# PraveenVora/pinot

Measured on AMD Instinct MI355X. Metric: rows/sec scanned + %HBM roofline, filter+GROUP BY SUM at 1/2/4/8 GPUs, higher is better.
Workload: dtype int64; 1 GPU; adanalytics_readme_query; rows_per_gpu=1000000000, segments_per_gpu=100, parallelism=segment-sharded dp1, RCCL reduce of partial aggregates, groups=8, matched_docs_rank0=118

## Files before the change

### include/pinot_amd.h

```cpp
#ifndef PINOT_AMD_H_
#define PINOT_AMD_H_

#include <stdint.h>

#ifdef __cplusplus
extern "C" {
#endif

#define PA_ABI_VERSION 5

#define PA_MAX_LEAVES 16
#define PA_MAX_OPS 48
#define PA_MAX_GROUP_BY 8
#define PA_MAX_AGGS 16
#define PA_MAX_ORDER_BY 8
#define PA_MAX_SELECT_COLUMNS 64
#define PA_MAX_SELECT_ROWS 65536
#define PA_MAX_AGG_FILTERS 8
#define PA_MAX_EXPRS 8
#define PA_MAX_EXPR_OPS 16
#define PA_MAX_EXPR_REGS 8
#define PA_MAX_EXPR_COLUMNS 8

#define PA_OK 0
// ... 344 lines not shown
                        void* stream);

int pa_query_key_layout(const pa_query* q, int32_t* hashed, int32_t* shifts);
int32_t pa_query_key_words(const pa_query* q);

int pa_query_stats(const pa_query* q, uint64_t* staged_bytes, uint64_t* num_docs,
                   uint64_t* num_tiles);

int32_t pa_query_column_staged(const pa_query* q, int32_t column_id);
int32_t pa_query_num_eager_literals(const pa_query* q);
int32_t pa_query_lane_major(const pa_query* q);
int32_t pa_query_dense_packed(const pa_query* q);
int32_t pa_query_count_free_emit(const pa_query* q);
int32_t pa_query_eq_prefilter(const pa_query* q);
int32_t pa_query_stream_nt(const pa_query* q);
int32_t pa_query_partition_keys(const pa_query* q);
int pa_query_plan(const pa_query* q, int32_t* strategy, int32_t* steps, int32_t* dma_slots, int32_t* ring,
                  int32_t* wg_per_cu, int32_t* grid, int32_t* lds_bytes);

void pa_query_destroy(pa_query* q);

#ifdef __cplusplus
}
#endif

#endif
```

### pinot_amd/_lib.py

```python
import ctypes
import os

HERE = os.path.dirname(os.path.abspath(__file__))
LIB_PATH = os.path.join(HERE, "libpinot_amd.so")

PA_MAX_LEAVES = 16
PA_MAX_OPS = 48
PA_MAX_GROUP_BY = 8
PA_MAX_AGGS = 16
PA_MAX_ORDER_BY = 8
PA_MAX_SELECT_COLUMNS = 64
PA_MAX_SELECT_ROWS = 65536
PA_MAX_AGG_FILTERS = 8
PA_MAX_EXPRS, PA_MAX_EXPR_OPS, PA_MAX_EXPR_REGS, PA_MAX_EXPR_COLUMNS = 8, 16, 8, 8
PA_EXPR_DOUBLE, PA_EXPR_LONG = 0, 1
PA_EXPR_ARG_REG, PA_EXPR_ARG_COL, PA_EXPR_ARG_F64, PA_EXPR_ARG_I64 = range(4)
PA_EXPR_LOAD_COL, PA_EXPR_ADD, PA_EXPR_SUB, PA_EXPR_MUL, PA_EXPR_DIV, PA_EXPR_MOD, PA_EXPR_ABS, PA_EXPR_CEIL, \
    PA_EXPR_FLOOR, PA_EXPR_D2L, PA_EXPR_L2D, PA_EXPR_TCONV_DIV, PA_EXPR_TCONV_MUL = range(13)

PA_OK, PA_EINVAL, PA_EHIP, PA_ENOMEM, PA_EUNSUPPORTED = 0, -1, -2, -3, -4
PA_INT, PA_LONG, PA_FLOAT, PA_DOUBLE, PA_STRING, PA_BYTES = range(6)
PA_LEAF_DICT_RANGE, PA_LEAF_DICT_SET, PA_LEAF_RAW_RANGE, PA_LEAF_MV_DICT_RANGE, PA_LEAF_MV_DICT_SET, PA_LEAF_RAW_SET = range(6)
PA_OP_LEAF, PA_OP_AND, PA_OP_OR, PA_OP_NOT = range(4)
PA_AGG_COUNT, PA_AGG_SUM, PA_AGG_MIN, PA_AGG_MAX, PA_AGG_DISTINCTCOUNTHLL, PA_AGG_COUNT_MV, PA_AGG_DISTINCTCOUNT, \
# ... 38 lines not shown
ABI_VERSION = 5

EXPORTED = [
    "pa_abi_version", "pa_device_count", "pa_set_device", "pa_last_error", "pa_host_alloc", "pa_host_free",
    "pa_segment_create", "pa_segment_add_sv_dict_column", "pa_segment_add_mv_dict_column",
    "pa_segment_add_raw_column", "pa_segment_num_docs", "pa_segment_device_bytes", "pa_segment_destroy",
    "pa_query_create", "pa_query_set_tuning", "pa_query_results_invalid", "pa_query_bind_segment",
    "pa_query_bind_value_remap", "pa_query_prepare", "pa_query_num_keys",
    "pa_query_set_selection", "pa_query_bind_order_remap", "pa_query_fetch_selection",
    "pa_query_selection_segment_docs", "pa_query_selection_counters",
    "pa_query_set_distinct", "pa_query_fetch_distinct",
    "pa_query_set_agg_filters", "pa_query_fetch_lane_counts", "pa_query_lane_docs",
    "pa_query_set_expressions",
    "pa_query_execute", "pa_query_reset", "pa_query_scan", "pa_query_num_eager_literals", "pa_query_lane_major",
    "pa_query_dense_packed", "pa_query_count_free_emit", "pa_query_eq_prefilter", "pa_query_stream_nt",
    "pa_query_partition_keys",
    "pa_query_accumulator_bytes", "pa_query_set_accumulator_buffer", "pa_query_num_sections", "pa_query_section",
    "pa_query_fetch", "pa_query_fetch_trimmed", "pa_query_fetch_histogram", "pa_query_percentiles",
    "pa_query_fetch_time_rows", "pa_query_time_row_form", "pa_query_matched_docs", "pa_query_key_layout", "pa_query_limit_trimming",
    "pa_query_num_groups_limit_reached", "pa_query_stats", "pa_query_leaf_bitmap_words", "pa_query_leaf_bitmaps",
    "pa_bitmap_counts_scratch_bytes", "pa_bitmap_counts", "pa_query_filter_counts",
    "pa_query_plan", "pa_query_column_staged", "pa_query_leap_leaf", "pa_query_leap_counts",
    "pa_query_execution_stats",
    "pa_query_row_bytes", "pa_query_pack_rows", "pa_query_merge_rows", "pa_query_key_words", "pa_query_destroy",
]


class PinotAmdError(RuntimeError):
    pass


# ... 132 lines not shown
        "pa_query_set_agg_filters": (ctypes.c_int, [vp, ctypes.POINTER(AggFilterSpec)]),
        "pa_query_fetch_lane_counts": (ctypes.c_int, [vp, vp, i64, vp]),
        "pa_query_lane_docs": (ctypes.c_int, [vp, vp]),
        "pa_query_set_expressions": (ctypes.c_int, [vp, ctypes.POINTER(ExprSpec)]),
        "pa_query_prepare": (ctypes.c_int, [vp]),
        "pa_query_num_keys": (i64, [vp]),
        "pa_query_execute": (ctypes.c_int, [vp, vp]),
        "pa_query_reset": (ctypes.c_int, [vp, vp]),
        "pa_query_scan": (ctypes.c_int, [vp, vp]),
        "pa_query_num_eager_literals": (i32, [vp]),
        "pa_query_lane_major": (i32, [vp]),
        "pa_query_dense_packed": (i32, [vp]),
        "pa_query_count_free_emit": (i32, [vp]),
        "pa_query_eq_prefilter": (i32, [vp]),
        "pa_query_stream_nt": (i32, [vp]),
        "pa_query_partition_keys": (i32, [vp]),
        "pa_query_accumulator_bytes": (u64, [vp]),
        "pa_query_set_accumulator_buffer": (ctypes.c_int, [vp, vp, u64]),
        "pa_query_num_sections": (i32, [vp]),
        "pa_query_section": (vp, [vp, i32, ctypes.POINTER(i32), ctypes.POINTER(i64)]),
        "pa_query_fetch": (i64, [vp, vp, i64, vp, vp, vp]),
        "pa_query_fetch_trimmed": (i64, [vp, vp, ctypes.POINTER(TrimSpec), i64, vp, vp, vp, ctypes.POINTER(i64)]),
        "pa_query_fetch_histogram": (i64, [vp, vp, i32, i64, i64, vp, vp, vp]),
        "pa_query_percentiles": (ctypes.c_int, [vp, vp, i32, i64, i32, vp, vp]),
        "pa_query_fetch_time_rows": (ctypes.c_int, [vp, vp, i32, i64, i32, vp, vp, vp, vp]),
        "pa_query_time_row_form": (i32, [vp, i32]),
        "pa_query_matched_docs": (i64, [vp]),
        "pa_query_key_layout": (ctypes.c_int, [vp, ctypes.POINTER(i32), ctypes.POINTER(i32)]),
        "pa_query_limit_trimming": (i32, [vp]),
        "pa_query_num_groups_limit_reached": (ctypes.c_int64, [vp]),
# ... 48 lines not shown
```

### pinot_amd/build.py

```python
import os
import re
import subprocess
import sys
import time
from concurrent.futures import ThreadPoolExecutor

HERE = os.path.dirname(os.path.abspath(__file__))
CSRC = os.path.join(HERE, "csrc")
LIB = os.path.join(HERE, "libpinot_amd.so")
SOURCES = ["pa_scan_lane_lm.hip", "pa_scan_std.hip", "pa_scan_part_mv.hip", "pa_scan_part_b.hip", "pa_scan_lane_raw.hip",
           "pa_scan_gdense.hip", "pa_scan_global.hip", "pa_scan_lane_dict.hip", "pa_kernels.hip", "pa_scan_part_a.hip",
           "pa_scan_filtered.hip", "pa_scan_expr.hip", "pa_scan_trow.hip", "pa_stats.hip", "pa_stats_host.hip", "pa_scan_lane_sm.hip", "pa_scan_distinct.hip",
           "pa_scan_select.hip", "pa_plan.hip",
           "pa_jit.hip", "pa_plan_kernels.hip", "pa_select.hip", "pa_distinct.hip", "pa_fetch.hip", "pa_capi.hip",
           "pa_compact.hip", "pa_segment.hip", "pa_hist.hip", "pa_prep.hip", "pa_launch_scan.hip", "pa_merge.hip",
           "pa_pve.hip", "pa_trim.hip"]
HEADERS = sorted(f for f in os.listdir(CSRC) if f.endswith(".h")) + [os.path.join("..", "..", "include", "pinot_amd.h")]
FLAGS = ["--offload-arch=gfx950", "-O3", "-fPIC", "-shared", "-munsafe-fp-atomics", "-std=c++17",
         "-Wall", "-Wno-unused-function"]
JIT_SOURCES = ["gdl_jit.hip", "pve_jit.hip"]
JIT_ABI = "pa_jit_abi.h"
_INCLUDE = re.compile(r'^\s*#\s*include\s+"([^"]+)"', re.M)


def _deps(path, seen=None):
    seen = set() if seen is None else seen
    if path in seen or not os.path.exists(path):
        return seen
    seen.add(path)
    for inc in _INCLUDE.findall(open(path, errors="replace").read()):
        for d in (os.path.dirname(path), CSRC, os.path.join(HERE, "..", "include")):
            cand = os.path.normpath(os.path.join(d, inc))
            if os.path.exists(cand):
                _deps(cand, seen)
                break
# ... 83 lines not shown
```

### pinot_amd/csrc/pa_capi.hip

```cpp
#include "pa_host.h"

extern "C" {

pa_query* pa_query_create(const pa_query_spec* spec, int32_t num_segments) {
  if (!spec || num_segments < 0) {
    fail(PA_EINVAL, "bad query spec");
    return nullptr;
  }
  if (spec->num_leaves < 0 || spec->num_leaves > PA_MAX_LEAVES || spec->num_ops < 0 || spec->num_ops > PA_MAX_OPS ||
      spec->num_group_by < 0 || spec->num_group_by > PA_MAX_GROUP_BY || spec->num_aggs < 0 ||
      spec->num_aggs > PA_MAX_AGGS) {
    fail(PA_EINVAL, "query spec counts out of range");
    return nullptr;
  }
  pa_query* q = new pa_query();
  q->spec = *spec;
  q->nseg = num_segments;
  q->segs.assign(num_segments, nullptr);
  q->leaf_params.resize(num_segments);
  q->luts.resize(num_segments);
  q->remaps.resize(num_segments);
  q->has_remap.resize(num_segments);
  q->vremaps.assign(num_segments, std::vector<std::vector<int32_t>>(spec->num_aggs));
  return q;
// ... 269 lines not shown
    rc = plan_limit_buffers(q, P, cus, total_tiles);
    if (rc) return rc;
  }
  rc = alloc_leaps(q, P);
  if (rc) return rc;
  rc = upload_descriptors(q);
  if (rc) return rc;
  if (q->trow_wide) {
    rc = dev_alloc(q->dq_pass2, sizeof(DevQuery));
    if (rc) return rc;
    DevQuery h2 = q->hq;
    h2.trow_pass = 2;
    PA_HIP(hipMemcpy(q->dq_pass2.p, &h2, sizeof(DevQuery), hipMemcpyHostToDevice));
  }
  if (!q->is_distinct) rc = jit_plan(q, P, cus);
  if (rc) return rc;
  if (q->is_distinct) {
    rc = distinct_plan(q);
    if (rc) return rc;
  }
  rc = pve_plan(q, P, cus);
  if (rc) return rc;
  PA_HIP(hipDeviceSynchronize());
  q->prepared = true;
  return PA_OK;
}

int64_t pa_query_num_keys(const pa_query* q) { return q ? q->num_keys : -1; }

int pa_query_reset(pa_query* q, void* stream) {
// ... 120 lines not shown
      PA_HIP(launch_scan(q->emit_h_strat, q->steps, 0, q->grid, q->emit_h_lds, (const DevQuery*)q->dq_h.p,
                         (const DevSeg*)q->dsegs.p, plans, ps, st));
    PA_HIP(launch_part_agg(q->part_vk, (const DevQuery*)q->dq.p, ps, q->hq.num_parts, q->hq.pv, q->hq.v_fmt <= V_FMT_ID,
                           q->tune.passc_v16, q->part_lds_c, st));
    PA_HIP(hipEventRecord(a->last, st));
    a->last_stream = st;
    a->used = true;
    return PA_OK;
  }
  if (q->jit_fn) {
    void* pa = q->jit_args.p;
    void* ps = q->jit_segs.p;
    void* params[] = {&pa, &ps};
    PA_HIP(hipModuleLaunchKernel(q->jit_fn, q->jit_grid, 1, 1, q->jit_waves * kWave, 1, 1, q->jit_lds, st, params,
                                 nullptr));
    return PA_OK;
  }
  PartScratch none{};
  PA_HIP(launch_scan(q->strategy, q->steps, q->lane_major, q->grid, q->lds_bytes, (const DevQuery*)q->dq.p,
                     (const DevSeg*)q->dsegs.p, (const LmSegPlan*)q->dplans.p, none, st));
  if (q->trow_wide)
    PA_HIP(launch_scan(q->strategy, q->steps, q->lane_major, q->grid, q->lds_bytes, (const DevQuery*)q->dq_pass2.p,
                       (const DevSeg*)q->dsegs.p, (const LmSegPlan*)q->dplans.p, none, st));
  q->leap_searched = false;
  return PA_OK;
}

int pa_query_execute(pa_query* q, void* stream) {
  const int rc = pa_query_reset(q, stream);
  return rc ? rc : pa_query_scan(q, stream);
// ... 80 lines not shown
  return q->sections[section].ptr;
}

int pa_query_stats(const pa_query* q, uint64_t* staged_bytes, uint64_t* num_docs, uint64_t* num_tiles) {
  if (!q) return fail(PA_EINVAL, "null query");
  if (staged_bytes) *staged_bytes = q->staged_bytes;
  if (num_docs) *num_docs = q->num_docs;
  if (num_tiles) *num_tiles = q->num_tiles;
  return PA_OK;
}

int pa_query_plan(const pa_query* q, int32_t* strategy, int32_t* steps, int32_t* dma_slots, int32_t* ring,
                  int32_t* wg_per_cu, int32_t* grid, int32_t* lds_bytes) {
  if (!q || !q->prepared) return fail(PA_EINVAL, "query not prepared");
  if (strategy)
    *strategy = q->jit_fn ? (q->jit_waves >= 16 ? STRAT_GDENSE_LM16 : STRAT_GDENSE_LM8)
                          : (q->partitioned ? STRAT_PEMIT : q->strategy);
  if (steps) *steps = q->steps;
  if (dma_slots) *dma_slots = q->dma_slots;
  if (ring) *ring = q->plan_ring;
  if (wg_per_cu) *wg_per_cu = q->plan_wg;
  if (grid) *grid = q->grid;
  if (lds_bytes) *lds_bytes = q->lds_bytes;
  return PA_OK;
}

int32_t pa_query_num_eager_literals(const pa_query* q) { return q && q->prepared ? q->num_eager : -1; }

int32_t pa_query_time_row_form(const pa_query* q, int32_t agg) {
  if (!q || !q->prepared || agg < 0 || agg >= q->spec.num_aggs) return -1;
  return q->trow_form[agg];
}

int32_t pa_query_lane_major(const pa_query* q) { return q && q->prepared ? q->lane_major : -1; }
int32_t pa_query_eq_prefilter(const pa_query* q) { return q && q->prepared ? q->eq_prefilter : -1; }
int32_t pa_query_stream_nt(const pa_query* q) { return q && q->prepared ? q->stream_nt : -1; }
int32_t pa_query_count_free_emit(const pa_query* q) { return q && q->prepared ? (q->pve.fn ? (q->pvh.fn ? 2 : 1) : 0) : -1; }
int32_t pa_query_partition_keys(const pa_query* q) {
  if (!q || !q->prepared) return -1;
  if (!q->partitioned || q->hq.pv == 0) return 0;
  return q->hq.part_kr_v ? q->hq.part_kr_v : (int32_t)1 << q->hq.kshift_v;
}
int32_t pa_query_dense_packed(const pa_query* q) {
  return q && q->prepared ? (q->jit_fn ? 2 : (q->dense_packed ? 1 : 0)) : -1;
}

int32_t pa_query_column_staged(const pa_query* q, int32_t column_id) {
  if (!q || !q->prepared || q->nseg == 0) return -1;
  for (size_t sl = 0; sl < q->slot_cols.size(); ++sl)
    if (q->slot_cols[sl] == column_id) {
      if (q->jit_fn) return std::count(q->jit_cols.begin(), q->jit_cols.end(), (int)sl) ? 1 : 0;
      return q->hsegs[0].cols[sl].lds_off >= 0 ? 1 : 0;
    }
  return -1;
}

int64_t pa_query_matched_docs(const pa_query* q) { return q && q->prepared ? q->last_matched : -1; }

int32_t pa_query_limit_trimming(const pa_query* q) {
// ... 19 lines not shown
```

### pinot_amd/csrc/pa_host.h

```cpp
#pragma once
#include <hip/hip_runtime.h>
#include <hip/hiprtc.h>

#include <algorithm>
#include <array>
#include <cstdio>
#include <cstdlib>
#include <cmath>
#include <cstring>
#include <functional>
#include <map>
#include <mutex>
#include <numeric>
#include <string>
#include <utility>
#include <vector>

#include "pa_device.h"
#include "pa_launch.h"
#include "pa_jit_abi.h"
#include "pa_tuning.h"

using namespace pa;

// ... 189 lines not shown

  DevQuery hq;
  std::vector<DevSeg> hsegs;
  DevBuf dq, dsegs, dplans;
  void* host_acc = nullptr;
  DevBuf fetch_blocks, fetch_stage;
  void* fetch_host = nullptr;
  DevBuf trim_buf;
  int lane_major = 0;
  int eq_prefilter = 0;
  int stream_nt = 0;
  int dense_packed = 0;
  hipFunction_t jit_fn = nullptr;
  int jit_waves = 0, jit_grid = 0, jit_lds = 0, jit_nd = 16, jit_nseg = 0, jit_classes = 0, jit_slots = 0;
  std::vector<int> jit_cols;
  DevBuf jit_args, jit_segs;
  struct PveStream {
    hipFunction_t fn = nullptr;
    int waves = 0, grid = 0, lds = 0, cr = 0, parts = 0, bin_shift = 5;
    int64_t chunks = 0;
    DevBuf args, segs, buf;
    size_t o_table = 0, o_hist = 0, o_used = 0, o_off = 0, o_base = 0, o_index = 0, o_tot = 0;
  } pve, pvh;
  int has_mv = 0;
  bool hashed = false;
  int key_words = 1;
  int64_t ht_slots = 0;
  int key_shift[PA_MAX_GROUP_BY] = {0};
  int keys_section = -1;
  bool partitioned = false;
// ... 200 lines not shown
int plan_scratch(pa_query* q, const Prep& P);
int plan_walk(pa_query* q, const Prep& P);
int plan_limit_buffers(pa_query* q, const Prep& P, int cus, int64_t total_tiles);
int upload_descriptors(pa_query* q);
PartScratch scratch_of(const pa_query* q, void* base);
size_t leap_header_bytes(const pa_query* q);
int plan_leaps(pa_query* q, const Prep& P);
int alloc_leaps(pa_query* q, const Prep& P);
int select_validate(pa_query* q);
int select_plan(pa_query* q);
int select_reset(pa_query* q, hipStream_t st);
int distinct_key_space(pa_query* q, Prep& P);
int distinct_plan(pa_query* q);
int jit_plan(pa_query* q, const Prep& P, int cus);
void jit_fill_pointers(pa_query* q, JitArgs& a);
void pve_fill_pointers(const pa_query::PveStream& st, unsigned long long* matched, PveArgs& a);
int pve_plan(pa_query* q, const Prep& P, int cus);
```

### pinot_amd/csrc/pa_jit.hip

```cpp
#include "pa_host.h"

static const char* kGdlJitSrc =
#include "gdl_jit_src.inc"
    ;

namespace {
std::mutex g_jit_mu;
struct JitEntry {
  hipModule_t mod = nullptr;
  hipFunction_t fn = nullptr;
};
std::map<std::string, JitEntry> g_jit_cache;

std::string int_list(const std::vector<int>& v) {
  std::string r = "{";
  for (size_t i = 0; i < v.size(); ++i) r += (i ? "," : "") + std::to_string(v[i]);
  return r + "}";
}

hipFunction_t jit_compile(const std::vector<std::string>& defs, const char* src = kGdlJitSrc,
                          const char* name = "gdl_jit") {
  int dev = 0;
  (void)hipGetDevice(&dev);
  std::string key = std::to_string(dev) + " " + name;
// ... 54 lines not shown

struct JitSum {
  int col = 0;
  int w = 0;
  bool table = false;
  bool shared = true;
  bool offs = false;
  int64_t base = 0, step = 1;
  std::vector<int64_t> aoff;
  int max_card = 0;
};
}

int jit_plan(pa_query* q, const Prep& P, int cus) {
  q->jit_fn = nullptr;
  q->jit_cols.clear();
  const pa_query_spec& s = q->spec;
  if (q->nseg == 0 || s.num_group_by != 1 || !P.gd_box_ok || P.gd_box || q->hq.leap_mode || q->partitioned ||
      q->limit_mode || q->limit_walk || q->hashed)
    return PA_OK;
  const Tuning& tn = q->tune;
  if ((s.flags & PA_QF_NO_JIT) || tn.debug_emit) return PA_OK;
  if (s.flags & (PA_QF_NO_DENSE_GROUP | PA_QF_FORCE_GLOBAL | PA_QF_FORCE_LDS | PA_QF_LAZY_POST | PA_QF_NO_LANE_MAJOR |
                 PA_QF_STEPS16 | PA_QF_DEBUG_STREAM_ONLY | PA_QF_NO_GDENSE_LM | PA_QF_NO_GD_PACK))
    return PA_OK;
  const int nl_all = (int)q->literals.size();
  if (q->num_eager != nl_all) return PA_OK;
  for (int li = 0; li < nl_all; ++li) {
    const int kind = s.leaves[q->literals[li].leaf].kind;
    if (kind != PA_LEAF_DICT_RANGE && kind != PA_LEAF_DICT_SET) return PA_OK;
// ... 435 lines not shown
  PA_HIP(hipMemcpy(q->jit_args.p, &a, sizeof(a), hipMemcpyHostToDevice));
  PA_HIP(hipMemcpy(q->jit_segs.p, js.data(), sizeof(JitSeg) * js.size(), hipMemcpyHostToDevice));
  q->jit_fn = fn;
  q->jit_waves = W;
  q->jit_nd = ND;
  q->jit_lds = (int)lds;
  q->jit_grid = G;
  q->jit_nseg = ni;
  q->jit_classes = (int)classes.size();
  q->jit_slots = nslot;
  q->jit_cols = cols;
  PLAN_LOG("gdl_jit: W %d ND %d RS %d RR %d ring %d lmax %d segdrain %d classes %zu slots %d (%zu B) segments %d/%d "
           "ktab %d kib %d lds %zu drain %d",
           W, ND, RS, RR, ring_n, lmax, (int)segdrain, classes.size(), nslot, slot_b, ni, q->nseg, (int)ktab, (int)kib,
           lds, drain);
  return PA_OK;
}

static const char* kPveJitSrc =
#include "pve_jit_src.inc"
    ;


void pve_fill_pointers(const pa_query::PveStream& st, unsigned long long* matched, PveArgs& a) {
  char* b = (char*)st.buf.p;
  a.recs = (uint32_t*)b;
  a.table = (uint32_t*)(b + st.o_table);
  a.hist = (uint32_t*)(b + st.o_hist);
  a.used = (uint32_t*)(b + st.o_used);
  a.matched = matched;
// ... 317 lines not shown
```

### pinot_amd/csrc/pa_jit_abi.h

```cpp
#pragma once

constexpr int kJitMax = 6;
constexpr int kJitMaxGb = 4;

struct JitSeg {
  unsigned long long src[kJitMax];
  long long first_tile;
  int num_docs, num_tiles;
  unsigned int lo_t[kJitMax], hi_t[kJitMax];
  int cls;
  int lbase, lspan;
  int gofs;
  int aoff[kJitMax];
  unsigned long long ktab;
  unsigned long long lut[kJitMax];
  unsigned long long tab[kJitMax];
  int lut_words[kJitMax];
  int tab_n[kJitMax];
  int ktab_n;
  unsigned int neg;
};
struct JitArgs {
  long long total_tiles;
  int nseg, nkeys, key_lo, key_span, xcd_major, pad;
  long long key_stride;
  unsigned long long* matched;
  unsigned long long* count;
  long long* sum[kJitMax];
  int sum_long[kJitMax];
  long long base[kJitMax], step[kJitMax];
};
static_assert(sizeof(JitSeg) == 48 + 8 + 8 + 48 + 16 + 24 + 8 + 48 + 48 + 24 + 24 + 8, "JitSeg layout");
static_assert(sizeof(JitArgs) == 8 + 24 + 8 + 8 + 8 + 48 + 24 + 48 + 48, "JitArgs layout");

struct PveSeg {
  unsigned long long src[kJitMax];
  long long first_tile;
  int num_docs, num_tiles;
  unsigned int lo_t[kJitMax], hi_t[kJitMax];
  unsigned long long admit;
  unsigned long long raw;
  unsigned long long mv_off;
  unsigned long long mv_words;
  unsigned long long hlut;
  int koff[kJitMaxGb];
  unsigned long long ktab[kJitMaxGb];
  int voff, vtab_n;
  unsigned long long vtab;
};
// ... 13 lines not shown
```

### pinot_amd/csrc/pa_tuning.h

```cpp
#pragma once
#include <cstdint>
#include <cstring>

#define PA_TUNINGS(X)                                                                                                  \
                                                                                  \
  X(gdl_w, -1, 8, 16, 0)                                                                                               \
  X(gdl_nd, -1, 8, 16, 0)                                                                                              \
  X(gdl_rs, -1, 1, 2, 0)                                                                                               \
                                                                                        \
  X(gdl_rr, -1, 1, 64, 0)                                                                                              \
                    \
  X(gdl_ring, -1, 2, 4, 0)                                                                                             \
         \
  X(gdl_dbg, 0, 0, 3, 1)                                                                                               \
                                      \
  X(pve_nd, -1, 8, 16, 0)                                                                                              \
         \
  X(pve_bs, -1, 16, 32, 0)                                                                                             \
                                                                              \
  X(pve_q, -1, 0, 1, 0)                                                                                                \
   \
  X(pve_ring, -1, 2, 4, 0)                                                                                             \
              \
  X(pve_hrun, -1, 0, 1, 0)                                                                                             \
                       \
  X(pve_hb, -1, 1, 8, 0)                                                                                               \
                                    \
  X(pve_dbg, 0, 0, 2, 1)                                                                                               \
                                                               \
  X(passc_v16, -1, 0, 1, 0)                                                                                            \
                                                                      \
  X(walk_tab, 1, 0, 1, 0)                                                                                              \
               \
  X(debug_emit, 0, 0, 127, 1)                                                                                          \
                                \
  X(eq_prefilter, -1, 0, 1, 0)                                                                                         \
                                                                                            \
  X(stream_nt, -1, 0, 1, 0)                                                                                            \
        \
  X(scan_grid, -1, 1, 4096, 0)                                                                                         \
                                                                    \
  X(reset_fused, -1, 0, 1, 0)                                                                                          \
         \
  X(select_scratch_mib, 256, 1, 16384, 0)                                                                              \
                                                    \
  X(select_cap, -1, 2, 131072, 0)                                                                                      \
     \
  X(distinct_lds, 1, 0, 2, 0)                                                                                          \
                                                                                 \
  X(filtered_lds, -1, 0, 1, 0)                                                                                         \
                                                    \
  X(expr_lds, -1, 0, 1, 0)                                                                                             \
    \
// ... 36 lines not shown
```

### pinot_amd/engine.py

```python
import ctypes
import dataclasses
import threading
from dataclasses import dataclass, field
from typing import Dict, List, Optional

import numpy as np

from . import _lib as L
from . import predicate as P
from . import query as Q
from . import transform as T
from .hll import HyperLogLog, hash_value
from .java_hash import java_hash_code
from .optimizer import optimize_filter
from .segment import Segment

_VTYPE = {"INT": L.PA_INT, "LONG": L.PA_LONG, "FLOAT": L.PA_FLOAT, "DOUBLE": L.PA_DOUBLE, "STRING": L.PA_STRING}


class UnsupportedQuery(L.PinotAmdError):
    pass


def column_ids_for(segment: Segment) -> Dict[str, int]:
# ... 699 lines not shown
        names = ("strategy", "steps", "dma_slots", "ring", "wg_per_cu", "grid", "lds_bytes")
        out["plan"] = {n: v.value for n, v in zip(names, vals)}
        code = out["plan"]["strategy"]
        out["plan"]["strategy"] = {0: "lds", 1: "global", 2: "partitioned", 4: "lane", 5: "lane", 6: "lane", 7: "lane",
                                    8: "lds_dense", 9: "lds_dense", 10: "lds_dense", 11: "lds_dense", 12: "lds_dense",
                                    14: "lds_dense", 15: "lds_dense", 128: "select", 129: "distinct",
                                    130: "distinct", 131: "filtered", 132: "filtered", 133: "expr", 134: "expr",
                                    135: "time_rows", 136: "time_rows"}[code]
        out["plan"]["variant"] = STRATEGY_VARIANTS.get(code, str(code))
        out["plan"]["eager_literals"] = int(L.lib().pa_query_num_eager_literals(self.handle))
        out["plan"]["lane_major"] = int(L.lib().pa_query_lane_major(self.handle))
        out["plan"]["dense_packed"] = int(L.lib().pa_query_dense_packed(self.handle))
        out["plan"]["count_free_emit"] = int(L.lib().pa_query_count_free_emit(self.handle))
        out["plan"]["eq_prefilter"] = int(L.lib().pa_query_eq_prefilter(self.handle))
        out["plan"]["stream_nt"] = int(L.lib().pa_query_stream_nt(self.handle))
        out["plan"]["partition_keys"] = int(L.lib().pa_query_partition_keys(self.handle))
        out["plan"]["limit_trimming"] = int(L.lib().pa_query_limit_trimming(self.handle))
        out["plan"]["results_invalid"] = int(L.lib().pa_query_results_invalid(self.handle))
        out["plan"]["time_row_form"] = {i: int(L.lib().pa_query_time_row_form(self.handle, i))
                                        for i, (t, _, _) in enumerate(self.pa_aggs) if t in TIME_ROW_AGGS}
        return out

    def fetch_arrays(self, stream=None, pooled=False, trim_spec=None):
        lib = L.lib()
        alloc = (lambda slot, n, dt: OUTPUT_POOL.array(slot, n, dt)) if pooled else (lambda slot, n, dt: np.empty(n, dt))
        cap = 1 if not self.query.group_by else min(self.num_keys, 1 << 16)
        if trim_spec is not None:
            cap = max(1, min(self.num_keys, int(trim_spec.trim)))
            total = ctypes.c_int64(0)
        elif self.query.group_by and self.num_keys > 1 << 16:
# ... 679 lines not shown
```

Before: 2580 billion rows/s.

## Add JIT-compiled equality-scan kernel with SWAR prefilter and lazy survivor aggregation

Adds a new JIT-compiled kernel, eqs_jit, for queries whose first leaf is an equality on a packed dictionary column and whose aggregates are int/long SUMs. Packed bit tiles stream into LDS through a ring of global_load_lds DMA buffers. A branch-free SWAR borrow trick tests whether any value in a word can match and skips tiles with no candidates. Only surviving docs decode the lazy leaves, group-by keys and sum columns straight from global memory and update them with atomics. The aim is to cut ALU and decode work on a very selective filter so the scan runs near HBM bandwidth, at the cost of extra planning, JIT compile time and a separate code path.

```diff
diff --git a/include/pinot_amd.h b/include/pinot_amd.h
--- a/include/pinot_amd.h
+++ b/include/pinot_amd.h
@@ -382,6 +382,7 @@
 int32_t pa_query_count_free_emit(const pa_query* q);
 int32_t pa_query_eq_prefilter(const pa_query* q);
 int32_t pa_query_stream_nt(const pa_query* q);
+int32_t pa_query_eq_jit(const pa_query* q);
 int32_t pa_query_partition_keys(const pa_query* q);
 int pa_query_plan(const pa_query* q, int32_t* strategy, int32_t* steps, int32_t* dma_slots, int32_t* ring,
                   int32_t* wg_per_cu, int32_t* grid, int32_t* lds_bytes);
diff --git a/pinot_amd/_lib.py b/pinot_amd/_lib.py
--- a/pinot_amd/_lib.py
+++ b/pinot_amd/_lib.py
@@ -76,7 +76,7 @@
     "pa_query_set_expressions",
     "pa_query_execute", "pa_query_reset", "pa_query_scan", "pa_query_num_eager_literals", "pa_query_lane_major",
     "pa_query_dense_packed", "pa_query_count_free_emit", "pa_query_eq_prefilter", "pa_query_stream_nt",
-    "pa_query_partition_keys",
+    "pa_query_eq_jit", "pa_query_partition_keys",
     "pa_query_accumulator_bytes", "pa_query_set_accumulator_buffer", "pa_query_num_sections", "pa_query_section",
     "pa_query_fetch", "pa_query_fetch_trimmed", "pa_query_fetch_histogram", "pa_query_percentiles",
     "pa_query_fetch_time_rows", "pa_query_time_row_form", "pa_query_matched_docs", "pa_query_key_layout", "pa_query_limit_trimming",
@@ -239,6 +239,7 @@
         "pa_query_count_free_emit": (i32, [vp]),
         "pa_query_eq_prefilter": (i32, [vp]),
         "pa_query_stream_nt": (i32, [vp]),
+        "pa_query_eq_jit": (i32, [vp]),
         "pa_query_partition_keys": (i32, [vp]),
         "pa_query_accumulator_bytes": (u64, [vp]),
         "pa_query_set_accumulator_buffer": (ctypes.c_int, [vp, vp, u64]),
diff --git a/pinot_amd/build.py b/pinot_amd/build.py
--- a/pinot_amd/build.py
+++ b/pinot_amd/build.py
@@ -18,7 +18,7 @@
 HEADERS = sorted(f for f in os.listdir(CSRC) if f.endswith(".h")) + [os.path.join("..", "..", "include", "pinot_amd.h")]
 FLAGS = ["--offload-arch=gfx950", "-O3", "-fPIC", "-shared", "-munsafe-fp-atomics", "-std=c++17",
          "-Wall", "-Wno-unused-function"]
-JIT_SOURCES = ["gdl_jit.hip", "pve_jit.hip"]
+JIT_SOURCES = ["gdl_jit.hip", "pve_jit.hip", "eqs_jit.hip"]
 JIT_ABI = "pa_jit_abi.h"
 _INCLUDE = re.compile(r'^\s*#\s*include\s+"([^"]+)"', re.M)
 
diff --git a/pinot_amd/csrc/eqs_jit.hip b/pinot_amd/csrc/eqs_jit.hip
--- /dev/null
+++ b/pinot_amd/csrc/eqs_jit.hip
@@ -0,0 +1,388 @@
+typedef unsigned int u32;
+typedef unsigned long long u64;
+typedef long long i64;
+typedef __attribute__((address_space(3))) u32 l32;
+typedef __attribute__((address_space(3))) u64 l64;
+typedef const __attribute__((address_space(1))) u32 g32;
+typedef const __attribute__((address_space(1))) int gi32;
+typedef const __attribute__((address_space(1))) i64 gi64;
+typedef __attribute__((address_space(1))) u64 gu64;
+
+#include "pa_jit_abi.h"
+
+#ifndef JIT_DBG
+#define JIT_DBG 0
+#endif
+constexpr int W = JIT_W, R = JIT_RING, IMG = JIT_IMG, NCLS = JIT_NCLS, NLZ = JIT_NLZ, NG = JIT_NG, NA = JIT_NA;
+constexpr int kNB[NCLS] = JIT_NB;
+constexpr int TD = 2048;
+constexpr u32 REG = 16;
+static_assert(R >= 2 && R <= 8, "2..8 tile images per wave");
+static_assert(NCLS >= 1 && NCLS <= 4, "1..4 width classes");
+static_assert(NLZ <= kJitMax && NG <= kJitMaxGb && NA <= kJitMax, "shape beyond the JIT descriptors");
+
+typedef const __attribute__((address_space(4))) JitArgs CA;
+typedef const __attribute__((address_space(4))) EqsHdr CH;
+typedef const __attribute__((address_space(4))) EqsSeg CS;
+
+__device__ __forceinline__ u32 lds_addr(const void* p) { return (u32)(unsigned long)(const l32*)p; }
+template <class T>
+__device__ __forceinline__ T* at(u32 a) { return (T*)(unsigned long)a; }
+
+template <int N>
+__device__ __forceinline__ void vm_wait() {
+  static_assert(N >= 0 && N < 64, "vmcnt is 6 bits");
+  asm volatile("s_waitcnt vmcnt(%0)" ::"n"(N) : "memory");
+}
+
+#if JIT_NT
+#define EQS_MOD " nt"
+#else
+#define EQS_MOD ""
+#endif
+__device__ __forceinline__ void dma16(u32 voff, u64 sbase, u32 dst) {
+  u32 keep;
+  asm volatile("s_mov_b32 %0, m0\n\ts_mov_b32 m0, %3\n\ts_nop 0\n\tglobal_load_lds_dwordx4 %1, %2" EQS_MOD
+               "\n\ts_mov_b32 m0, %0"
+               : "=&s"(keep) : "v"(voff), "s"(sbase), "s"(dst));
+}
+__device__ __forceinline__ void dma16m(u32 voff, u64 sbase, u32 dst, u64 mask) {
+  u32 keep;
+  u64 save;
+  asm volatile(
+      "s_mov_b64 %1, exec\n\ts_mov_b64 exec, %5\n\ts_mov_b32 %0, m0\n\ts_mov_b32 m0, %4\n\ts_nop 0\n\t"
+      "global_load_lds_dwordx4 %2, %3" EQS_MOD "\n\ts_mov_b32 m0, %0\n\ts_mov_b64 exec, %1"
+      : "=&s"(keep), "=&s"(save) : "v"(voff), "s"(sbase), "s"(dst), "s"(mask));
+}
+
+constexpr int dma_instrs(int nb) { return (16 * nb + 63) / 64; }
+constexpr int dma_max() {
+  int n = 0;
+  for (int k = 0; k < NCLS; ++k) n = dma_instrs(kNB[k]) > n ? dma_instrs(kNB[k]) : n;
+  return n;
+}
+constexpr int D = dma_max();
+static_assert((R - 2) * D < 64, "the counted wait must fit vmcnt");
+
+template <int K>
+__device__ __forceinline__ void dma_tile_k(u64 src, int wt, u32 img, u32 voff) {
+  constexpr int NB = kNB[K];
+  constexpr int CH = 16 * NB;
+  const u64 s = src + (u64)(u32)wt * (u64)(256 * NB);
+  const u32 dst = img + REG;
+#pragma unroll
+  for (int k = 0; k < CH / 64; ++k) dma16(voff, s + 1024u * k, dst + 1024u * k);
+  if constexpr (CH % 64) dma16m(voff, s + 1024u * (CH / 64), dst + 1024u * (CH / 64), (1ull << (CH % 64)) - 1ull);
+#pragma unroll
+  for (int k = dma_instrs(NB); k < D; ++k) dma16m(voff, src, img, 1ull);
+}
+template <int K>
+__device__ __forceinline__ void dma_tile(int cls, u64 src, int wt, u32 img, u32 voff) {
+  if constexpr (K + 1 < NCLS) {
+    if (cls == K) dma_tile_k<K>(src, wt, img, voff);
+    else dma_tile<K + 1>(cls, src, wt, img, voff);
+  } else {
+    dma_tile_k<K>(src, wt, img, voff);
+  }
+}
+
+template <int NB>
+constexpr u32 eq_low_bits(int w) {
+  u32 m = 0;
+  for (int i = 0; i < 32; ++i) {
+    const int s = (i + 1) * NB - 1;
+    if ((s >> 5) == w) m |= 0x80000000u >> (s & 31);
+  }
+  return m;
+}
+template <int NB>
+constexpr u32 eq_high_bits(int w) {
+  u32 m = 0;
+  for (int i = 0; i < 32; ++i) {
+    const int s = i * NB;
+    if ((s >> 5) == w) m |= 0x80000000u >> (s & 31);
+  }
+  return m;
+}
+template <int NB>
+__device__ __forceinline__ u32 eq_pattern_word(u64 window, int j) {
+  return (u32)((window << ((32 * j) % NB)) >> 32);
+}
+template <int NB, int J>
+__device__ __forceinline__ void eq_any_word(const u32 (&p)[NB], const u32 (&pat)[NB], u64& borrow, u32& any) {
+  constexpr u32 L = eq_low_bits<NB>(J), H = eq_high_bits<NB>(J);
+  const u32 x = p[J] ^ pat[J];
+  u32 d;
+  asm("v_subb_co_u32_e64 %[d], %[b], %[x], %[l], %[b]" : [d] "=v"(d), [b] "+s"(borrow) : [x] "v"(x), [l] "v"(L));
+  any |= d & ~x & H;
+  if constexpr (J > 0) eq_any_word<NB, J - 1>(p, pat, borrow, any);
+}
+
+template <int NB>
+__device__ __forceinline__ u32 leaf_eq(const u32 (&w)[NB], u32 lo_t, u32 hi_t) {
+  u32 nm = 0;
+#pragma unroll
+  for (int i = 31; i >= 0; --i) {
+    const int s = i * NB, j = s >> 5, o = s & 31;
+    const u32 t = (o + NB <= 32) ? (w[j] << o) : __builtin_amdgcn_alignbit(w[j], w[j + 1 < NB ? j + 1 : j], 32 - o);
+    u32 u;
+    asm("v_sub_u32_e64 %[u], %[t], %[lo]\n\tv_sub_co_u32_e32 %[u], vcc, %[hi], %[u]\n\t"
+        "v_addc_co_u32_e32 %[nm], vcc, %[nm], %[nm], vcc"
+        : [nm] "+v"(nm), [u] "=&v"(u) : [t] "v"(t), [lo] "s"(lo_t), [hi] "s"(hi_t) : "vcc");
+  }
+  return ~nm;
+}
+
+__device__ __forceinline__ u32 decode_global(u64 words, i64 doc, int nb) {
+  const u64 e1 = (u64)doc * (u64)nb + (u64)(nb - 1);
+  const i64 we = (i64)(e1 >> 5);
+  const u32 lo = ((g32*)words)[we];
+  const u32 hi = ((g32*)words)[we - 1];
+  return __builtin_amdgcn_alignbit(hi, lo, (~(u32)e1) & 31u) & (nb >= 32 ? 0xffffffffu : ((1u << nb) - 1u));
+}
+
+__device__ __forceinline__ u32 leap_tile(CH* Hd, int si, i64 doc_base, u32 e, u32 f, int lane, u32 slice, u32 listed,
+                                         u32 lds_base) {
+  const u32 mine = (u32)__builtin_popcount(e);
+  u32 incl = mine;
+#pragma unroll
+  for (int o = 1; o < 64; o <<= 1) {
+    const u32 t = (u32)__shfl_up((int)incl, o, 64);
+    if (lane >= o) incl += t;
+  }
+  const u32 total = (u32)__builtin_amdgcn_readlane((int)incl, 63);
+  u32 matched = (u32)__builtin_popcount(f);
+#pragma unroll
+  for (int o = 1; o < 64; o <<= 1) matched += (u32)__shfl_xor((int)matched, o, 64);
+  const i64 nseg = Hd->nseg;
+  const u64 cap = (u64)Hd->leap_cap;
+  gu64* out = (gu64*)Hd->leap_out;
+  if ((u64)listed + total > cap) {
+    if (lane == 0) __hip_atomic_fetch_or(out + 3 * nseg, 1ull, __ATOMIC_RELAXED, __HIP_MEMORY_SCOPE_AGENT);
+  } else {
+    gu64* list = out + 3 * nseg + 1 + Hd->leap_slices + (i64)slice * (i64)cap;
+    const u32 lcap = (u32)Hd->leap_lds_cap;
+    u32 pos = listed + (incl - mine);
+    while (e) {
+      const int i = __builtin_ctz(e);
+      e &= e - 1u;
+      const i64 doc = doc_base + 32 * lane + i;
+      const u64 ent = ((u64)si << 40) | ((u64)doc << 1) | ((f >> i) & 1u);
+      if (pos < lcap) at<l64>(lds_base)[pos] = ent;
+      else list[pos] = ent;
+      ++pos;
+    }
+  }
+  if (lane == 0 && matched)
+    __hip_atomic_fetch_add(out + 3 * (i64)si, (u64)matched, __ATOMIC_RELAXED, __HIP_MEMORY_SCOPE_AGENT);
+  return listed + total;
+}
+
+struct Surv {
+  u32 matched, listed;
+};
+
+__device__ __noinline__ Surv survivors(CA* A, CH* Hd, CS* sg, i64 doc_base, u32 m, int lane, u32 slice, u32 listed,
+                                       u32 leap_lds) {
+  if constexpr (NLZ > 0) {
+    const u32 eager = m;
+#pragma unroll 1
+    for (int i = 0; i < 32; ++i) {
+      const u32 bit = 1u << i;
+      if (__builtin_amdgcn_ballot_w64((m & bit) != 0) == 0) continue;
+      const i64 doc = doc_base + 32 * lane + i;
+      bool ok = (m & bit) != 0;
+#pragma unroll
+      for (int l = 0; l < NLZ; ++l) {
+        if (ok) {
+          const u32 id = decode_global(sg->lazy[l].words, doc, sg->lazy[l].nb);
+          ok = ((id - sg->lazy[l].lo) < sg->lazy[l].span) != (sg->lazy[l].neg != 0);
+        }
+      }
+      if (!ok) m &= ~bit;
+    }
+    if constexpr (JIT_LEAP) listed = leap_tile(Hd, sg->index, doc_base, eager, m, lane, slice, listed, leap_lds);
+  }
+  if (__builtin_amdgcn_ballot_w64(m != 0) != 0) {
+#pragma unroll 1
+    for (int i = 0; i < 32; ++i) {
+      const u32 bit = 1u << i;
+      if (__builtin_amdgcn_ballot_w64((m & bit) != 0) == 0) continue;
+      if ((m & bit) == 0) continue;
+      const i64 doc = doc_base + 32 * lane + i;
+      i64 key = 0;
+#pragma unroll
+      for (int j = 0; j < NG; ++j) {
+        u32 id = decode_global(sg->gb[j].words, doc, sg->gb[j].nb);
+        if (sg->gb[j].tab != 0) id = (u32)((gi32*)sg->gb[j].tab)[id];
+        key += (i64)((u64)id * (u64)Hd->gb_stride[j]);
+      }
+      __hip_atomic_fetch_add((gu64*)A->count + key, 1ull, __ATOMIC_RELAXED, __HIP_MEMORY_SCOPE_AGENT);
+#pragma unroll
+      for (int a = 0; a < NA; ++a) {
+        const u32 id = decode_global(sg->sum[a].words, doc, sg->sum[a].nb);
+        const i64 v = ((gi64*)sg->sum[a].tab)[id];
+        gu64* acc = (gu64*)A->sum[a];
+        if (A->sum_long[a]) {
+          __hip_atomic_fetch_add(acc + 2 * key, (u64)(u32)v, __ATOMIC_RELAXED, __HIP_MEMORY_SCOPE_AGENT);
+          __hip_atomic_fetch_add(acc + 2 * key + 1, (u64)(v >> 32), __ATOMIC_RELAXED, __HIP_MEMORY_SCOPE_AGENT);
+        } else {
+          __hip_atomic_fetch_add(acc + key, (u64)v, __ATOMIC_RELAXED, __HIP_MEMORY_SCOPE_AGENT);
+        }
+      }
+    }
+  }
+  vm_wait<0>();
+  return Surv{(u32)__builtin_popcount(m), listed};
+}
+
+__device__ __forceinline__ int find_segment(CS* segs, int nseg, int t) {
+  int lo = 0, hi = nseg - 1;
+  while (lo < hi) {
+    const int mid = (lo + hi + 1) >> 1;
+    if (segs[mid].first_tile <= t) lo = mid;
+    else hi = mid - 1;
+  }
+  while (t >= segs[lo].first_tile + segs[lo].num_tiles) ++lo;
+  return lo;
+}
+
+struct Walk {
+  CA* A;
+  CH* Hd;
+  CS* S;
+  int t, t1, ti;
+  int isi;
+  int ifirst, iend;
+  u64 isrc;
+  int icls;
+  u32 ring, voff;
+  int slot;
+  int lane;
+  u32 slice, listed, leap_lds, matched;
+};
+
+__device__ __forceinline__ void issue(Walk& w, int to) {
+  if (w.ti < w.t1) {
+    while (w.ti >= w.iend) {
+      ++w.isi;
+      w.ifirst = (int)w.S[w.isi].first_tile;
+      w.iend = w.ifirst + w.S[w.isi].num_tiles;
+      w.isrc = w.S[w.isi].src;
+      w.icls = w.S[w.isi].cls;
+    }
+    dma_tile<0>(w.icls, w.isrc, w.ti - w.ifirst, w.ring + (u32)to * (u32)(IMG * 4), w.voff);
+  }
+  ++w.ti;
+}
+
+template <int K>
+__device__ __forceinline__ void run(Walk& w, CS* sg, int end) {
+  constexpr int NB = kNB[K];
+  const int first = (int)sg->first_tile;
+  const int full_end = first + sg->num_docs / TD;
+  const int num_docs = sg->num_docs;
+  const u32 lo_t = sg->lo_t, hi_t = sg->hi_t;
+  const u64 win = sg->win;
+  u32 pat[NB];
+#pragma unroll
+  for (int j = 0; j < NB; ++j) pat[j] = eq_pattern_word<NB>(win, j);
+  const u32 lane_words = REG + (u32)w.lane * (u32)(NB * 4);
+  for (; w.t < end; ++w.t) {
+    if (R > 2 && w.t + (R - 2) < w.t1) vm_wait<(R > 2 ? (R - 2) * D : 0)>();
+    else vm_wait<0>();
+    issue(w, w.slot == 0 ? R - 1 : w.slot - 1);
+    const u32 img = w.ring + (u32)w.slot * (u32)(IMG * 4);
+    w.slot = w.slot + 1 == R ? 0 : w.slot + 1;
+    if constexpr (JIT_DBG == 1) continue;
+    const l32* p = at<const l32>(img + lane_words);
+    u32 wv[NB];
+#pragma unroll
+    for (int j = 0; j < NB; ++j) wv[j] = p[j];
+    u32 any = 0;
+    u64 borrow = 0;
+    eq_any_word<NB, NB - 1>(wv, pat, borrow, any);
+    if (__builtin_amdgcn_ballot_w64(any != 0) == 0) continue;
+    u32 m = leaf_eq<NB>(wv, lo_t, hi_t);
+    if (w.t >= full_end) {
+      const i64 n = (i64)num_docs - (i64)(w.t - first) * TD - 32 * w.lane;
+      m &= n >= 32 ? 0xffffffffu : (n <= 0 ? 0u : ((1u << n) - 1u));
+    }
+    if (__builtin_amdgcn_ballot_w64(m != 0) == 0) continue;
+    const Surv s = survivors(w.A, w.Hd, sg, (i64)(w.t - first) * TD, m, w.lane, w.slice, w.listed, w.leap_lds);
+    w.matched += s.matched;
+    w.listed = (u32)__builtin_amdgcn_readfirstlane((int)s.listed);
+  }
+}
+template <int K>
+__device__ __forceinline__ void run_any(int cls, Walk& w, CS* sg, int end) {
+  if constexpr (K + 1 < NCLS) {
+    if (cls == K) run<K>(w, sg, end);
+    else run_any<K + 1>(cls, w, sg, end);
+  } else {
+    run<K>(w, sg, end);
+  }
+}
+
+extern "C" __global__ void __launch_bounds__(W * 64, JIT_WG) eqs_jit(const JitArgs* a_in, const EqsHdr* h_in) {
+  CA* A = (CA*)(unsigned long)a_in;
+  CH* Hd = (CH*)(unsigned long)h_in;
+  CS* S = (CS*)(unsigned long)(h_in + 1);
+  extern __shared__ __attribute__((aligned(16))) u32 smem[];
+  const u32 base = lds_addr(smem);
+  const int lane = threadIdx.x & 63;
+  const int wave = __builtin_amdgcn_readfirstlane(threadIdx.x >> 6);
+  const i64 T = A->total_tiles, G = gridDim.x;
+  const i64 b = blockIdx.x;
+  const i64 lb = A->xcd_major ? (b % 8) * (G / 8) + (b % 8 < G % 8 ? b % 8 : G % 8) + b / 8 : b;
+  const i64 gw = lb * W + wave, NW = G * W;
+  Walk w;
+  w.A = A;
+  w.Hd = Hd;
+  w.S = S;
+  w.t = (int)(gw * T / NW);
+  w.t1 = (int)((gw + 1) * T / NW);
+  w.lane = lane;
+  w.ring = base + (u32)wave * (u32)(R * IMG * 4);
+  w.voff = 16u * (u32)lane;
+  w.slot = 0;
+  w.slice = (u32)gw;
+  w.listed = 0;
+  w.matched = 0;
+  w.leap_lds = base + (u32)(W * R * IMG * 4) + (u32)wave * (u32)Hd->leap_lds_cap * 8u;
+  if (w.t < w.t1) {
+    const int nseg = A->nseg;
+    int si = find_segment(S, nseg, w.t);
+    w.isi = si;
+    w.ifirst = (int)S[si].first_tile;
+    w.iend = w.ifirst + S[si].num_tiles;
+    w.isrc = S[si].src;
+    w.icls = S[si].cls;
+    w.ti = w.t;
+#pragma unroll
+    for (int k = 0; k + 1 < R; ++k) issue(w, k);
+    while (w.t < w.t1) {
+      CS* sg = S + si;
+      const int seg_end = (int)sg->first_tile + sg->num_tiles;
+      run_any<0>(sg->cls, w, sg, seg_end < w.t1 ? seg_end : w.t1);
+      if (w.t < w.t1) {
+        ++si;
+        while (w.t >= S[si].first_tile + S[si].num_tiles) ++si;
+      }
+    }
+    vm_wait<0>();
+  }
+  if constexpr (JIT_LEAP) {
+    gu64* out = (gu64*)Hd->leap_out;
+    const i64 nseg = Hd->nseg;
+    const u32 lcap = (u32)Hd->leap_lds_cap;
+    const u32 nl = w.listed < lcap ? w.listed : lcap;
+    gu64* list = out + 3 * nseg + 1 + Hd->leap_slices + (i64)w.slice * Hd->leap_cap;
+    for (u32 k = (u32)lane; k < nl; k += 64) list[k] = at<const l64>(w.leap_lds)[k];
+    if (lane == 0) out[3 * nseg + 1 + w.slice] = w.listed;
+  }
+  u64 wm = w.matched;
+#pragma unroll
+  for (int o = 32; o > 0; o >>= 1) wm += __shfl_xor(wm, o);
+  if (lane == 0 && wm) __hip_atomic_fetch_add((gu64*)A->matched, wm, __ATOMIC_RELAXED, __HIP_MEMORY_SCOPE_AGENT);
+}
diff --git a/pinot_amd/csrc/pa_capi.hip b/pinot_amd/csrc/pa_capi.hip
--- a/pinot_amd/csrc/pa_capi.hip
+++ b/pinot_amd/csrc/pa_capi.hip
@@ -307,6 +307,7 @@
     PA_HIP(hipMemcpy(q->dq_pass2.p, &h2, sizeof(DevQuery), hipMemcpyHostToDevice));
   }
   if (!q->is_distinct) rc = jit_plan(q, P, cus);
+  if (!rc) rc = eqs_plan(q, P, cus);
   if (rc) return rc;
   if (q->is_distinct) {
     rc = distinct_plan(q);
@@ -457,6 +458,7 @@
     void* params[] = {&pa, &ps};
     PA_HIP(hipModuleLaunchKernel(q->jit_fn, q->jit_grid, 1, 1, q->jit_waves * kWave, 1, 1, q->jit_lds, st, params,
                                  nullptr));
+    if (q->eq_jit) q->leap_searched = false;
     return PA_OK;
   }
   PartScratch none{};
@@ -567,7 +569,7 @@
                   int32_t* wg_per_cu, int32_t* grid, int32_t* lds_bytes) {
   if (!q || !q->prepared) return fail(PA_EINVAL, "query not prepared");
   if (strategy)
-    *strategy = q->jit_fn ? (q->jit_waves >= 16 ? STRAT_GDENSE_LM16 : STRAT_GDENSE_LM8)
+    *strategy = q->jit_fn && !q->eq_jit ? (q->jit_waves >= 16 ? STRAT_GDENSE_LM16 : STRAT_GDENSE_LM8)
                           : (q->partitioned ? STRAT_PEMIT : q->strategy);
   if (steps) *steps = q->steps;
   if (dma_slots) *dma_slots = q->dma_slots;
@@ -588,6 +590,7 @@
 int32_t pa_query_lane_major(const pa_query* q) { return q && q->prepared ? q->lane_major : -1; }
 int32_t pa_query_eq_prefilter(const pa_query* q) { return q && q->prepared ? q->eq_prefilter : -1; }
 int32_t pa_query_stream_nt(const pa_query* q) { return q && q->prepared ? q->stream_nt : -1; }
+int32_t pa_query_eq_jit(const pa_query* q) { return q && q->prepared ? q->eq_jit : -1; }
 int32_t pa_query_count_free_emit(const pa_query* q) { return q && q->prepared ? (q->pve.fn ? (q->pvh.fn ? 2 : 1) : 0) : -1; }
 int32_t pa_query_partition_keys(const pa_query* q) {
   if (!q || !q->prepared) return -1;
@@ -595,7 +598,7 @@
   return q->hq.part_kr_v ? q->hq.part_kr_v : (int32_t)1 << q->hq.kshift_v;
 }
 int32_t pa_query_dense_packed(const pa_query* q) {
-  return q && q->prepared ? (q->jit_fn ? 2 : (q->dense_packed ? 1 : 0)) : -1;
+  return q && q->prepared ? (q->jit_fn && !q->eq_jit ? 2 : (q->dense_packed ? 1 : 0)) : -1;
 }
 
 int32_t pa_query_column_staged(const pa_query* q, int32_t column_id) {
diff --git a/pinot_amd/csrc/pa_host.h b/pinot_amd/csrc/pa_host.h
--- a/pinot_amd/csrc/pa_host.h
+++ b/pinot_amd/csrc/pa_host.h
@@ -227,6 +227,7 @@
   hipFunction_t jit_fn = nullptr;
   int jit_waves = 0, jit_grid = 0, jit_lds = 0, jit_nd = 16, jit_nseg = 0, jit_classes = 0, jit_slots = 0;
   std::vector<int> jit_cols;
+  int eq_jit = 0;
   DevBuf jit_args, jit_segs;
   struct PveStream {
     hipFunction_t fn = nullptr;
@@ -457,5 +458,6 @@
 int distinct_plan(pa_query* q);
 int jit_plan(pa_query* q, const Prep& P, int cus);
 void jit_fill_pointers(pa_query* q, JitArgs& a);
+int eqs_plan(pa_query* q, const Prep& P, int cus);
 void pve_fill_pointers(const pa_query::PveStream& st, unsigned long long* matched, PveArgs& a);
 int pve_plan(pa_query* q, const Prep& P, int cus);
diff --git a/pinot_amd/csrc/pa_jit.hip b/pinot_amd/csrc/pa_jit.hip
--- a/pinot_amd/csrc/pa_jit.hip
+++ b/pinot_amd/csrc/pa_jit.hip
@@ -1,4 +1,5 @@
 #include "pa_host.h"
+#include "pa_eq_any.h"
 
 static const char* kGdlJitSrc =
 #include "gdl_jit_src.inc"
@@ -92,6 +93,7 @@
 
 int jit_plan(pa_query* q, const Prep& P, int cus) {
   q->jit_fn = nullptr;
+  q->eq_jit = 0;
   q->jit_cols.clear();
   const pa_query_spec& s = q->spec;
   if (q->nseg == 0 || s.num_group_by != 1 || !P.gd_box_ok || P.gd_box || q->hq.leap_mode || q->partitioned ||
@@ -557,6 +559,153 @@
            "ktab %d kib %d lds %zu drain %d",
            W, ND, RS, RR, ring_n, lmax, (int)segdrain, classes.size(), nslot, slot_b, ni, q->nseg, (int)ktab, (int)kib,
            lds, drain);
+  return PA_OK;
+}
+
+static const char* kEqsJitSrc =
+#include "eqs_jit_src.inc"
+    ;
+constexpr int kEqJitMinCard = 4096;
+
+int eqs_plan(pa_query* q, const Prep& P, int cus) {
+  (void)cus;
+  q->eq_jit = 0;
+  if (q->jit_fn) return PA_OK;
+  const pa_query_spec& s = q->spec;
+  const Tuning& tn = q->tune;
+  const DevQuery& h = q->hq;
+  if (tn.eq_jit == 0 || (s.flags & (PA_QF_NO_JIT | PA_QF_DEBUG_STREAM_ONLY)) || tn.debug_emit) return PA_OK;
+  if (q->nseg == 0 || q->num_tiles == 0 || q->num_tiles >= (uint64_t(1) << 31) || q->strategy != STRAT_GLOBAL || !q->lane_major || q->steps != 32 ||
+      q->hashed || q->partitioned || q->limit_mode || q->limit_walk || q->has_mv || h.gb_mv >= 0 || q->is_select ||
+      q->is_distinct || q->is_filtered || q->is_expr || q->is_trow)
+    return PA_OK;
+  const int nl = (int)q->literals.size(), ng = s.num_group_by;
+  if (nl < 1 || nl - 1 > kJitMax || q->num_eager < 1 || ng > kJitMaxGb || h.num_gb != ng) return PA_OK;
+  for (int li = 0; li < nl; ++li)
+    if (!q->clause_end[li] || s.leaves[q->literals[li].leaf].kind != PA_LEAF_DICT_RANGE) return PA_OK;
+  std::vector<int> sums;
+  for (int a = 0; a < s.num_aggs; ++a) {
+    if (s.aggs[a].type == PA_AGG_COUNT) continue;
+    if (s.aggs[a].type != PA_AGG_SUM || (h.aggs[a].src != SRC_INT && h.aggs[a].src != SRC_LONG)) return PA_OK;
+    sums.push_back(a);
+  }
+  const int na = (int)sums.size();
+  if (na > kJitMax) return PA_OK;
+  auto dict_col = [](const DevCol& c) { return c.kind == COL_SV_DICT && c.words && c.nbits >= 1 && c.nbits <= 32; };
+  const int slot0 = P.leaf_slot[q->literals[0].leaf];
+  std::vector<int> classes, seg_cls(q->nseg, 0);
+  int min_card = INT32_MAX, nb_max = 0;
+  for (int si = 0; si < q->nseg; ++si) {
+    const DevSeg& d = q->hsegs[si];
+    const DevLeaf& L = d.leaves[0];
+    const DevCol& c0 = d.cols[slot0];
+    const int nb = c0.nbits;
+    if (d.admit || !dict_col(c0) || nb > kEqPrefilterMaxNb || L.kind != PA_LEAF_DICT_RANGE || L.negate ||
+        L.nbits != nb || (uint32_t)L.span != (uint32_t)((uint64_t(1) << (32 - nb)) - 1))
+      return PA_OK;
+    for (int li = 1; li < nl; ++li)
+      if (d.leaves[li].kind != PA_LEAF_DICT_RANGE || !dict_col(d.cols[P.leaf_slot[q->literals[li].leaf]])) return PA_OK;
+    for (int j = 0; j < ng; ++j)
+      if (!dict_col(d.cols[h.gb_slot[j]])) return PA_OK;
+    for (int a : sums)
+      if (!dict_col(d.cols[h.aggs[a].slot]) || !d.cols[h.aggs[a].slot].dict_i64) return PA_OK;
+    min_card = std::min(min_card, (int)c0.card);
+    nb_max = std::max(nb_max, nb);
+    auto it = std::find(classes.begin(), classes.end(), nb);
+    if (it == classes.end()) {
+      if (classes.size() == 4) return PA_OK;
+      classes.push_back(nb);
+      it = classes.end() - 1;
+    }
+    seg_cls[si] = (int)(it - classes.begin());
+  }
+  if (tn.eq_jit < 0 && min_card < kEqJitMinCard) return PA_OK;
+  const int W = scan_waves(STRAT_GLOBAL), R = h.ring;
+  int dmax = 0;
+  for (int nb : classes) dmax = std::max(dmax, (16 * nb + 63) / 64);
+  if (R < 2 || R > 8 || (R - 2) * dmax >= 64) return PA_OK;
+  const size_t img = al16((size_t)16 + (size_t)256 * nb_max + 16);
+  const size_t lds = (size_t)W * R * img + (h.leap_mode ? (size_t)W * h.leap_lds_cap * 8 : 0);
+  const int wg = std::max(1, std::min(4, q->plan_wg));
+  if (lds * (size_t)wg > kLdsBudget) return PA_OK;
+  std::vector<std::string> defs = {
+      "-DJIT_W=" + std::to_string(W), "-DJIT_WG=" + std::to_string(wg), "-DJIT_RING=" + std::to_string(R),
+      "-DJIT_IMG=" + std::to_string(img / 4), "-DJIT_NCLS=" + std::to_string(classes.size()),
+      "-DJIT_NB=" + int_list(classes), "-DJIT_NT=" + std::to_string(q->stream_nt ? 1 : 0),
+      "-DJIT_NLZ=" + std::to_string(nl - 1), "-DJIT_NG=" + std::to_string(ng), "-DJIT_NA=" + std::to_string(na),
+      "-DJIT_LEAP=" + std::to_string(h.leap_mode ? 1 : 0)};
+  if (tn.eqs_dbg) defs.push_back("-DJIT_DBG=" + std::to_string(tn.eqs_dbg));
+  hipFunction_t fn = jit_compile(defs, kEqsJitSrc, "eqs_jit");
+  if (!fn) return PA_OK;
+  (void)hipFuncSetAttribute((const void*)fn, hipFuncAttributeMaxDynamicSharedMemorySize, (int)lds);
+  JitArgs a;
+  std::memset(&a, 0, sizeof(a));
+  a.total_tiles = h.total_wtiles;
+  a.nseg = q->nseg;
+  a.xcd_major = h.xcd_major;
+  jit_fill_pointers(q, a);
+  std::vector<char> buf(sizeof(EqsHdr) + sizeof(EqsSeg) * (size_t)q->nseg, 0);
+  EqsHdr& hd = *(EqsHdr*)buf.data();
+  EqsSeg* js = (EqsSeg*)(buf.data() + sizeof(EqsHdr));
+  hd.leap_out = h.leap_out;
+  hd.leap_cap = h.leap_cap;
+  hd.leap_slices = h.leap_slices;
+  hd.leap_lds_cap = h.leap_mode ? h.leap_lds_cap : 0;
+  hd.nseg = q->nseg;
+  for (int j = 0; j < ng; ++j) hd.gb_stride[j] = h.gb_stride[j];
+  for (int si = 0; si < q->nseg; ++si) {
+    const DevSeg& d = q->hsegs[si];
+    EqsSeg& j = js[si];
+    const DevLeaf& L = d.leaves[0];
+    const int nb = d.cols[slot0].nbits;
+    j.src = (unsigned long long)(uintptr_t)d.cols[slot0].words;
+    j.first_tile = d.first_wtile;
+    j.num_docs = d.num_docs;
+    j.num_tiles = d.num_wtiles;
+    j.lo_t = (uint32_t)L.lo;
+    j.hi_t = (uint32_t)L.span;
+    j.win = eq_pattern_window(nb, (uint32_t)L.lo >> (32 - nb));
+    j.cls = seg_cls[si];
+    j.index = d.index;
+    for (int li = 1; li < nl; ++li) {
+      const DevLeaf& Z = d.leaves[li];
+      const DevCol& c = d.cols[P.leaf_slot[q->literals[li].leaf]];
+      const int sh = 32 - c.nbits;
+      EqsLeaf& z = j.lazy[li - 1];
+      z.words = (unsigned long long)(uintptr_t)c.words;
+      z.lo = (uint32_t)Z.lo >> sh;
+      z.span = (uint32_t)(((uint64_t)(uint32_t)Z.span + 1u) >> sh);
+      z.nb = c.nbits;
+      z.neg = Z.negate ? 1 : 0;
+    }
+    for (int g = 0; g < ng; ++g) {
+      const DevCol& c = d.cols[h.gb_slot[g]];
+      j.gb[g].words = (unsigned long long)(uintptr_t)c.words;
+      j.gb[g].tab = (unsigned long long)(uintptr_t)d.remap[g];
+      j.gb[g].nb = c.nbits;
+    }
+    for (int k = 0; k < na; ++k) {
+      const DevCol& c = d.cols[h.aggs[sums[k]].slot];
+      j.sum[k].words = (unsigned long long)(uintptr_t)c.words;
+      j.sum[k].tab = (unsigned long long)(uintptr_t)c.dict_i64;
+      j.sum[k].nb = c.nbits;
+    }
+  }
+  int rc = dev_alloc(q->jit_args, sizeof(JitArgs));
+  if (!rc) rc = dev_alloc(q->jit_segs, buf.size());
+  if (rc) return rc;
+  PA_HIP(hipMemcpy(q->jit_args.p, &a, sizeof(a), hipMemcpyHostToDevice));
+  PA_HIP(hipMemcpy(q->jit_segs.p, buf.data(), buf.size(), hipMemcpyHostToDevice));
+  q->jit_fn = fn;
+  q->eq_jit = 1;
+  q->jit_waves = W;
+  q->jit_lds = (int)lds;
+  q->jit_grid = q->grid;
+  q->jit_nseg = q->nseg;
+  q->jit_classes = (int)classes.size();
+  q->jit_cols.assign(1, slot0);
+  PLAN_LOG("eqs_jit: W %d grid %d ring %d classes %zu nt %d lazy %d gb %d sums %d leap %d lds %zu", W, q->grid, R,
+           classes.size(), q->stream_nt, nl - 1, ng, na, h.leap_mode, lds);
   return PA_OK;
 }
 
diff --git a/pinot_amd/csrc/pa_jit_abi.h b/pinot_amd/csrc/pa_jit_abi.h
--- a/pinot_amd/csrc/pa_jit_abi.h
+++ b/pinot_amd/csrc/pa_jit_abi.h
@@ -33,6 +33,37 @@
 static_assert(sizeof(JitSeg) == 48 + 8 + 8 + 48 + 16 + 24 + 8 + 48 + 48 + 24 + 24 + 8, "JitSeg layout");
 static_assert(sizeof(JitArgs) == 8 + 24 + 8 + 8 + 8 + 48 + 24 + 48 + 48, "JitArgs layout");
 
+struct EqsLeaf {
+  unsigned long long words;
+  unsigned int lo, span;
+  int nb, neg;
+};
+struct EqsCol {
+  unsigned long long words;
+  unsigned long long tab;
+  int nb, pad;
+};
+struct EqsSeg {
+  unsigned long long src;
+  long long first_tile;
+  int num_docs, num_tiles;
+  unsigned int lo_t, hi_t;
+  unsigned long long win;
+  int cls, index;
+  EqsLeaf lazy[kJitMax];
+  EqsCol gb[kJitMaxGb];
+  EqsCol sum[kJitMax];
+};
+struct EqsHdr {
+  unsigned long long* leap_out;
+  long long leap_cap, leap_slices;
+  int leap_lds_cap, nseg;
+  long long gb_stride[kJitMaxGb];
+};
+static_assert(sizeof(EqsLeaf) == 24 && sizeof(EqsCol) == 24, "EqsLeaf / EqsCol layout");
+static_assert(sizeof(EqsSeg) == 48 + 24 * (kJitMax + kJitMaxGb + kJitMax), "EqsSeg layout");
+static_assert(sizeof(EqsHdr) == 32 + 8 * kJitMaxGb, "EqsHdr layout");
+
 struct PveSeg {
   unsigned long long src[kJitMax];
   long long first_tile;
diff --git a/pinot_amd/csrc/pa_tuning.h b/pinot_amd/csrc/pa_tuning.h
--- a/pinot_amd/csrc/pa_tuning.h
+++ b/pinot_amd/csrc/pa_tuning.h
@@ -37,6 +37,10 @@
   X(eq_prefilter, -1, 0, 1, 0)                                                                                         \
                                                                                             \
   X(stream_nt, -1, 0, 1, 0)                                                                                            \
+                 \
+  X(eq_jit, -1, 0, 1, 0)                                                                                               \
+                    \
+  X(eqs_dbg, 0, 0, 1, 1)                                                                                               \
         \
   X(scan_grid, -1, 1, 4096, 0)                                                                                         \
                                                                     \
diff --git a/pinot_amd/engine.py b/pinot_amd/engine.py
--- a/pinot_amd/engine.py
+++ b/pinot_amd/engine.py
@@ -737,6 +737,7 @@
         out["plan"]["count_free_emit"] = int(L.lib().pa_query_count_free_emit(self.handle))
         out["plan"]["eq_prefilter"] = int(L.lib().pa_query_eq_prefilter(self.handle))
         out["plan"]["stream_nt"] = int(L.lib().pa_query_stream_nt(self.handle))
+        out["plan"]["eq_jit"] = int(L.lib().pa_query_eq_jit(self.handle))
         out["plan"]["partition_keys"] = int(L.lib().pa_query_partition_keys(self.handle))
         out["plan"]["limit_trimming"] = int(L.lib().pa_query_limit_trimming(self.handle))
         out["plan"]["results_invalid"] = int(L.lib().pa_query_results_invalid(self.handle))
```

Result: faster. 2778 billion rows/s (median of 6 runs) (+7.7%).
